# ugovaretto-accel/cuda-mpi-scratch

Hardware: AMD Instinct MI355X
Metric: 2D stencil Gcells/sec (higher is better)
Workload: dtype fp32

## Files before the change

### csrc/include/mxs/kernels/chunk_schedule.hpp

```cpp
#pragma once

#include <algorithm>
#include <cstdint>
#include <stdexcept>
#include <string>
#include <vector>

namespace mxs {
namespace kernels {

struct PassChunk {
  std::int32_t group = 0;
  std::int32_t r0 = 0, r1 = 0;
  std::int32_t pad = 0;
};

struct ChunkSchedule {
  int blocks = 0;
  int entries = 0;
  double bulk_cost = 0;
  std::vector<PassChunk> table;
  const PassChunk& at(int wg, int e) const { return table[size_t(wg) * size_t(entries) + size_t(e)]; }
};

// ... 9 lines not shown
  for (int w = 0; w < blocks && ri < runs.size(); ++w) {
    std::int64_t b = budget(w);
    while (b > fill && ri < runs.size()) {
      const std::int64_t take = std::min(b - fill, runs[ri].r1 - pos);
      emit(w, runs[ri].g, pos, pos + take);
      pos += take;
      b -= take + fill;
      if (pos == runs[ri].r1 && ++ri < runs.size()) pos = runs[ri].r0;
    }
  }
  std::int64_t left = 0;
  for (size_t i = ri; i < runs.size(); ++i) left += runs[i].r1 - (i == ri ? pos : runs[i].r0);
  return left;
}
template <typename BudgetT>
std::int64_t min_budget(const std::vector<Run>& runs, int blocks, std::int64_t fill, BudgetT budget_t) {
  std::int64_t total = 0;
  for (const auto& r : runs) total += r.r1 - r.r0;
  std::int64_t lo = 0, hi = total + 4 * fill + 1;
  auto ok = [&](std::int64_t T) {
    return greedy_walk(runs, blocks, fill, [&](int w) { return budget_t(w, T); },
                       [](int, std::int32_t, std::int64_t, std::int64_t) {}) == 0;
  };
  while (!ok(hi)) hi *= 2;
  while (lo + 1 < hi) {
    const std::int64_t mid = lo + (hi - lo) / 2;
    (ok(mid) ? hi : lo) = mid;
  }
  return hi;
}
}

inline std::vector<std::int64_t> balanced_starts(std::int64_t groups, std::int64_t rows, int blocks,
                                                 std::int64_t fill) {
  std::vector<detail::Run> runs;
  for (std::int64_t g = 0; g < groups; ++g) runs.push_back(detail::Run{std::int32_t(g), 0, rows});
  const std::int64_t T = detail::min_budget(runs, blocks, fill, [](int, std::int64_t t) { return t; });
  std::vector<std::int64_t> start(size_t(blocks) + 1, groups * rows);
  std::vector<std::uint8_t> seen(size_t(blocks), 0);
  detail::greedy_walk(runs, blocks, fill, [&](int) { return T; },
                      [&](int w, std::int32_t g, std::int64_t r0, std::int64_t) {
                        if (!seen[size_t(w)]) {
                          seen[size_t(w)] = 1;
                          start[size_t(w)] = std::int64_t(g) * rows + r0;
                        }
                      });
  for (int w = blocks - 1; w >= 0; --w)
    if (!seen[size_t(w)]) start[size_t(w)] = start[size_t(w) + 1];
  return start;
}

struct HaloLastSchedule {
  ChunkSchedule inner;
  ChunkSchedule outer;
  std::int64_t hf = 0;
  double inner_cost = 0, outer_cost = 0;
  double serial_cost = 0;
  std::int64_t band = 0;
  std::int64_t moved_rows = 0;
};

namespace detail {
inline ChunkSchedule partition_runs(const std::vector<Run>& runs, int blocks, std::int64_t fill, double* cost) {
  ChunkSchedule s;
  s.blocks = blocks;
  std::vector<std::vector<PassChunk>> lists(static_cast<size_t>(blocks));
  std::vector<std::int64_t> load(static_cast<size_t>(blocks), 0);
  if (!runs.empty()) {
    const std::int64_t T = min_budget(runs, blocks, fill, [](int, std::int64_t t) { return t; });
    greedy_walk(runs, blocks, fill, [&](int) { return T; },
                [&](int w, std::int32_t g, std::int64_t r0, std::int64_t r1) {
// ... 151 lines not shown
```

### csrc/include/mxs/kernels/kernels.hpp

```cpp
#pragma once

#include <hip/hip_runtime_api.h>

#include <cmath>
#include <cstdint>
#include <limits>

#include "mxs/grid/layout.hpp"
#include "mxs/kernels/chunk_schedule.hpp"
#include "mxs/kernels/fixed_edge_split.hpp"

namespace mxs {
namespace kernels {

template <typename T>
void fill(T* p, index_t n, T value, hipStream_t s);
template <typename T>
void fill_region(T* base, const Array2D& region, T value, hipStream_t s);
template <typename T>
void fill_random(T* tile, const TileGeom& g, index_t global_x0, index_t global_y0,
                 index_t global_width, std::uint64_t seed, T lo, T hi, hipStream_t s);

struct Stencil5Coeffs {
  double center = 0.2;
// ... 65 lines not shown
  int lag1 = 0;
  int blocks = 0;
  index_t groups = 0;
  index_t owg = 0;
  index_t fill = 0;
  index_t read_lead = 0, read_span = 0;
};
template <typename T>
bool chunk_pass_shape(const TileGeom& g, int steps, const Stencil5Coeffs& c, ChunkPassShape* out);
template <typename T>
void stencil5_chunk_pass(const T* in, T* out, const TileGeom& g, const Stencil5Coeffs& c, const ChunkPassShape& shape,
                         const PassChunk* table, int entries, hipStream_t s);

template <typename T>
void absmax(const T* x, index_t n, T* out, hipStream_t s);
bool streams_concurrent(hipStream_t a, hipStream_t b);
void spin_delay(double us, hipStream_t s);
constexpr int kClockStampWgs = 512;
void clock_stamp(unsigned long long* out, hipStream_t s);
void count_diff(const void* a, const void* b, index_t bytes, unsigned* out, hipStream_t s);

template <typename T>
void stencil5_rect(const T* in, T* out, const TileGeom& g, index_t x0, index_t x1, index_t y0,
                   index_t y1, Stencil5Coeffs c, hipStream_t s);

void set_gpu_share(int processes);
int gpu_share();

void set_pipe_joint(bool on);
bool pipe_joint();
void set_pipe_lag1(bool on);
bool pipe_lag1();
bool last_pipe_lag1();
void set_pipe_balanced(bool on);
bool pipe_balanced_on();

const char* last_stencil_dispatch();

constexpr int kMaxBoxRadius = 2;
struct BoxWeights {
  int radius = 1;
  float w[(2 * kMaxBoxRadius + 1) * (2 * kMaxBoxRadius + 1)] = {};
};
template <typename T>
void stencil_box(const T* in, T* out, const TileGeom& g, index_t x0, index_t x1, index_t y0,
                 index_t y1, const BoxWeights& w, hipStream_t s);

constexpr int kMaxCopies = 24;
struct Copy2D {
  index_t src_off = 0, src_stride = 0;
  index_t dst_off = 0, dst_stride = 0;
  index_t width = 0, height = 0;
  int src_slot = 0, dst_slot = 0;
};
struct Copy2DBatch {
  int n = 0;
  Copy2D op[kMaxCopies];
};
enum class CopyKind : int { Copy = 0, Pack = 1, Unpack = 2 };
template <typename T>
void copy2d_batch(T* slot0, T* slot1, T* slot2, const Copy2DBatch& b, hipStream_t s, int grid_x = 0, int block = 0,
                  CopyKind kind = CopyKind::Copy);

enum class DotReduce : int {
  Atomic = 0,
  TwoPass = 1,
// ... 15 lines not shown
```

### csrc/kernels/stencil.hip

```cpp
#include <hip/hip_runtime.h>

#include <algorithm>
#include <atomic>
#include <cmath>
#include <limits>
#include <cstdlib>
#include <string>
#include <vector>

#include "mxs/core/error.hpp"
#include "mxs/kernels/kernels.hpp"
#include "mxs/runtime/hip_utils.hpp"

#include "stencil_device.hpp"
#include "stencil_pipe.hpp"

namespace mxs {
namespace kernels {
namespace {
using namespace detail;
constexpr int kLdsRows = 16;

std::atomic<const char*> g_last_dispatch{"none"};
std::atomic<bool> g_last_lag1{false};
inline void note(const char* k) {
  g_last_dispatch.store(k, std::memory_order_relaxed);
  g_last_lag1.store(false, std::memory_order_relaxed);
}

template <typename T, int ROWS>
void launch_roll(const T* in, T* out, const TileGeom& g, index_t row_begin, index_t row_end, T c0, T c1,
                 hipStream_t s) {
  constexpr int N = Vec16<T>::N;
  constexpr int WX = 4, NW = 4;
  const index_t rows = row_end - row_begin;
  const index_t gx = (g.width + index_t(kWaveSize) * N * WX - 1) / (index_t(kWaveSize) * N * WX);
  const index_t gy = (rows + ROWS - 1) / ROWS;
  stencil5_roll_kernel<T, ROWS, ROWS, true, WX, false, NW><<<dim3(unsigned(gx), unsigned(gy)), NW * kWaveSize, 0, s>>>(
      in, out, g.pitch, g.core_offset(), g.width, row_begin, row_end, c0, c1);
}

}

template <typename T>
void stencil5_rows(const T* in, T* out, const TileGeom& g, index_t row_begin, index_t row_end,
                   Stencil5Coeffs c, hipStream_t s, StencilVariant v) {
  if (row_end <= row_begin || g.width <= 0) return;
  MXS_CHECK(g.halo_x >= 1 && g.halo_y >= 1, "stencil5 needs a ghost ring of at least 1");
  MXS_CHECK(row_begin >= 0 && row_end <= g.height, "row range out of the core");
  constexpr int N = Vec16<T>::N;
  MXS_CHECK((g.pitch % N) == 0 && ((g.x_origin + g.halo_x) % N) == 0,
            "stencil5_rows needs a TileGeom::aligned layout (16-byte aligned core rows)");
  MXS_CHECK(g.pitch >= g.x_origin + g.halo_x + ((g.width + N - 1) / N) * N + N,
            "pitch too small for vector loads");
  const T c0 = T(c.center), c1 = T(c.neighbor);
  const index_t rows = row_end - row_begin;
  const index_t gx = (g.width + kWaveSize * N - 1) / (kWaveSize * N);
  if (v == StencilVariant::LdsTile) {
    const index_t gy = (rows + kLdsRows - 1) / kLdsRows;
    const size_t lds = size_t(kLdsRows + 2) * (kWaveSize * N + 2 * N) * sizeof(T);
// ... 202 lines not shown
  stencil5_rect_kernel<T><<<unsigned(blocks), kBlock, 0, s>>>(in, out, g.pitch, g.core_offset(), x0, x1 - x0, y0,
                                                              y1 - y0, T(c.center), T(c.neighbor));
  note("rect");
  MXS_HIP_CHECK_LAUNCH();
}

template <typename T>
void stencil_box(const T* in, T* out, const TileGeom& g, index_t x0, index_t x1, index_t y0, index_t y1,
                 const BoxWeights& w, hipStream_t s) {
  if (x1 <= x0 || y1 <= y0) return;
  MXS_CHECK(w.radius == 1 || w.radius == 2, "box radius must be 1 or 2");
  MXS_CHECK(g.halo_x >= w.radius && g.halo_y >= w.radius, "ghost ring narrower than the box radius");
  const dim3 grid(unsigned((x1 - x0 + 63) / 64), unsigned((y1 - y0 + 15) / 16));
  if (w.radius == 1)
    stencil_box_kernel<T, 1><<<grid, kBlock, 0, s>>>(in, out, g.pitch, g.core_offset(), x0, x1 - x0, y0, y1 - y0, w);
  else
    stencil_box_kernel<T, 2><<<grid, kBlock, 0, s>>>(in, out, g.pitch, g.core_offset(), x0, x1 - x0, y0, y1 - y0, w);
  note("box");
  MXS_HIP_CHECK_LAUNCH();
}

const char* last_stencil_dispatch() { return g_last_dispatch.load(std::memory_order_relaxed); }

namespace {
std::atomic<int> g_gpu_share{1};
std::atomic<bool> g_pipe_joint{[] {
  const char* e = experiment_env("MXS_PIPE_JOINT");
  return !(e && std::string(e) == "0");
}()};
std::atomic<bool> g_pipe_lag1{[] {
  const char* e = experiment_env("MXS_PIPE_LAG1");
  return !(e && std::string(e) == "0");
}()};
std::atomic<bool> g_pipe_balanced{[] {
  const char* e = experiment_env("MXS_PIPE_BALANCED");
  return !(e && std::string(e) == "0");
}()};
}
void set_gpu_share(int processes) { g_gpu_share.store(std::max(1, processes), std::memory_order_relaxed); }
int gpu_share() { return g_gpu_share.load(std::memory_order_relaxed); }
void set_pipe_joint(bool on) { g_pipe_joint.store(on, std::memory_order_relaxed); }
bool pipe_joint() { return g_pipe_joint.load(std::memory_order_relaxed); }
void set_pipe_lag1(bool on) { g_pipe_lag1.store(on, std::memory_order_relaxed); }
bool pipe_lag1() { return g_pipe_lag1.load(std::memory_order_relaxed); }
bool last_pipe_lag1() { return g_last_lag1.load(std::memory_order_relaxed); }
void set_pipe_balanced(bool on) { g_pipe_balanced.store(on, std::memory_order_relaxed); }
bool pipe_balanced_on() { return g_pipe_balanced.load(std::memory_order_relaxed); }
namespace detail {
bool pipe_balanced() { return g_pipe_balanced.load(std::memory_order_relaxed); }
void pipe_starts(index_t groups, index_t rows, int blocks, index_t fill, PipeShares* out) {
  struct Entry {
    index_t groups, rows, fill;
    int blocks;
    std::vector<std::int64_t> start;
  };
  thread_local std::vector<Entry> cache;
  const Entry* hit = nullptr;
  for (const auto& e : cache)
    if (e.groups == groups && e.rows == rows && e.fill == fill && e.blocks == blocks) hit = &e;
  if (!hit) {
    if (cache.size() >= 16) cache.erase(cache.begin());
    cache.push_back(Entry{groups, rows, fill, blocks, balanced_starts(groups, rows, blocks, fill)});
    hit = &cache.back();
  }
  out->n = blocks;
  for (int w = 0; w <= blocks; ++w) out->start[w] = int(hit->start[size_t(w)]);
}
void note_dispatch(const char* k) { note(k); }
void note_pipe_lag1(bool lag1) { g_last_lag1.store(lag1, std::memory_order_relaxed); }
}

#define MXS_INST_STENCIL(T)                                                                                    \
  template void stencil5_rows<T>(const T*, T*, const TileGeom&, index_t, index_t, Stencil5Coeffs, hipStream_t, \
                                 StencilVariant);                                                              \
  template void stencil5_rect<T>(const T*, T*, const TileGeom&, index_t, index_t, index_t, index_t,             \
                                 Stencil5Coeffs, hipStream_t);                                                 \
  template void stencil5_periodic<T>(const T*, T*, const TileGeom&, Stencil5Coeffs, hipStream_t);              \
  template void stencil5_tb<T>(const T*, T*, const TileGeom&, int, index_t, index_t, index_t, index_t,          \
                               Stencil5Coeffs, bool, hipStream_t, StencilVariant);                             \
  template bool stencil5_periodic_supported<T>(const TileGeom&);                                               \
  template void stencil_box<T>(const T*, T*, const TileGeom&, index_t, index_t, index_t, index_t,               \
                               const BoxWeights&, hipStream_t);
MXS_INST_STENCIL(float)
MXS_INST_STENCIL(double)

}
}
```

### csrc/kernels/stencil_device.hpp

```cpp
#pragma once

#include <hip/hip_runtime.h>

#include "mxs/kernels/kernels.hpp"

namespace mxs {
namespace kernels {
namespace detail {

template <typename T>
struct Vec16 {
  static constexpr int N = 16 / sizeof(T);
  using type = T __attribute__((ext_vector_type(N)));
};

template <typename T>
__device__ __forceinline__ T fma_t(T a, T b, T c);
template <>
__device__ __forceinline__ float fma_t<float>(float a, float b, float c) { return __builtin_fmaf(a, b, c); }
template <>
__device__ __forceinline__ double fma_t<double>(double a, double b, double c) { return __builtin_fma(a, b, c); }

template <typename T>
__device__ __forceinline__ T jac(T c, T n, T s, T w, T e, T c0, T c1) {
// ... 897 lines not shown
    if (xw < x_end) {
      wp.done = a - a0;
      if constexpr (ROT)
        stream_chunk_fast<typename FastBody<T, SUM, XB>::type, S, PF, WRAP>(in, out, pitch, core_off, W, H, xw, x_end,
                                                                        y_begin + r0, y_begin + r1, c0, c1, &wp);
      else
        stream_chunk<T, S, PF, WRAP, DPP>(in, out, pitch, core_off, W, H, xw, x_end, y_begin + r0, y_begin + r1, c0,
                                          c1);
    }
    a += r1 - r0;
  }
}

template <int S0, int S1, int PF>
struct PipeShape {
  static constexpr int S = S0 + S1;
  static constexpr int RING = 3 * PF;
  static constexpr int T1 = (3 * S0 + PF - 1 + PF - 1) / PF;
};

template <int S0, int S1, int G>
struct JointShape {
  static constexpr int A0 = (S0 + 3) / 4 * 4, A1 = (S1 + 3) / 4 * 4;
  static constexpr int OW0 = 256 - 2 * A0;
  static constexpr int OW1 = 256 - 2 * A1;
  static constexpr int SPAN = G * OW0;
  static constexpr int OWG = SPAN - 2 * A1 < G * OW1 ? SPAN - 2 * A1 : G * OW1;
  static constexpr int ROW = G * kWaveSize;
  static constexpr int LEAD = A0 + A1;
  static_assert((G - 1) * OW1 + 256 <= 4 * ROW, "stage-1 windows must stay inside the joint row");
  static_assert(OWG > 0, "time block too deep for a joint group");
};

template <typename B, int S0, int S1, int PF, bool WRAP, bool JOINT = false, int G = kWavesPerBlock, int LAG1 = 0>
__device__ __forceinline__ void pipe_chunk(const typename B::T* __restrict__ in, typename B::T* __restrict__ out,
                                           index_t pitch, index_t core_off, index_t W, index_t H, index_t xw,
                                           index_t x_end, index_t ys, index_t ye, typename B::T c0, typename B::T c1,
                                           typename B::V* __restrict__ ring, int stage, int strip = 0) {
  static_assert(PF % 3 == 0, "the window rotates through 3 slots: PF must be a multiple of 3");
  using P = PipeShape<S0, S1, PF>;
  constexpr int S = P::S, RING = P::RING;
  using T = typename B::T;
  using V = typename B::V;
  using Sh = StripShape<T, S, true>;
  using J = JointShape<S0, S1, G>;
  constexpr bool ASC0 = (LAG1 & 1) != 0, ASC1 = (LAG1 & 2) != 0;
  constexpr int E0 = ASC0 ? 2 * S0 : 3 * S0 - 1, E1 = ASC1 ? 2 * S1 : 3 * S1 - 1;
  constexpr int N = Sh::N, SA = Sh::SA, AL = SA / N;
  static_assert(!JOINT || N == 4, "joint windows assume 4-cell lanes");
  const int lane = threadIdx.x & (kWaveSize - 1);
  const index_t gx = JOINT ? (stage == 0 ? xw - J::LEAD + index_t(strip) * J::OW0 : xw - J::A1 + index_t(strip) * J::OW1) +
                                 index_t(lane) * N
                           : xw - SA + index_t(lane) * N;
  const index_t rows = ye - ys;
  constexpr int D = (PF - E0 % PF) % PF;
  constexpr int T1 = (E0 + D) / PF + 1;
  static_assert(ASC0 || T1 == P::T1, "stage-1 start block");
  const index_t n_it0 = rows + 2 * S1 + E0 + D;
  const index_t n_it1 = rows + E1;
  const index_t blocks0 = (n_it0 + PF - 1) / PF, blocks1 = T1 + (n_it1 + PF - 1) / PF;
  const index_t blocks = blocks0 > blocks1 ? blocks0 : blocks1;
  constexpr int RSTRIDE = JOINT ? J::ROW : kWaveSize;
  int slot = lane;
  if constexpr (JOINT) {
    constexpr int AL0 = J::A0 / 4;
    if (stage == 0) {
      const bool valid = lane >= AL0 && lane < kWaveSize - AL0;
      const int tail = J::SPAN / 4 + strip * 2 * AL0 + (lane < AL0 ? lane : lane - (kWaveSize - 2 * AL0));
      slot = valid ? strip * (J::OW0 / 4) + lane - AL0 : tail;
    } else {
      slot = strip * (J::OW1 / 4) + lane;
    }
  }
  V* __restrict__ my = ring + slot;

  if (stage == 0) {
    index_t lx;
    if (!JOINT && xw >= x_end) {
      lx = 0;
    } else if constexpr (WRAP) {
      if (W >= (JOINT ? G : 1) * kWaveSize * N) lx = gx < 0 ? gx + W : (gx >= W ? gx - W : gx);
      else lx = ((gx % W) + W) % W;
    } else {
      const index_t last_col = (W + N - 1) / N * N + SA - N;
      lx = gx < last_col ? gx : last_col;
    }
    const T* __restrict__ pin = in + core_off + lx;
    const index_t last_row = ye + S - 1;
    V pf[PF];
#pragma unroll
    for (int k = 0; k < PF; ++k) {
      index_t r = ys - S - D + k;
      if constexpr (WRAP) r = r < 0 ? r + H : r;
      else r = r < ys - S ? ys - S : r;
      pf[k] = B::load(pin + r * pitch);
    }
    index_t next = ys - S - D + PF;
    if constexpr (WRAP) next = next < 0 ? next + H : next;
    index_t roff = next * pitch;
    auto fetch = [&]() -> V {
      const V v = B::load(pin + roff);
// ... 55 lines not shown
            if (l == S0 - 1) top = v;
            else win[n][l + 1] = v;
          }
        } else {
          const int p0 = k % 3, p1 = (k + 1) % 3, p2 = (k + 2) % 3;
          win[p2][0] = B::enter(pf[k]);
          pf[k] = fetch();
#pragma unroll
          for (int l = S0 - 1; l >= 0; --l) {
            const V o = B::jac(win[p0][l], win[p1][l], win[p2][l], c0, c1);
            if (l == S0 - 1) top = o;
            else win[p0][l + 1] = o;
          }
        }
        my[(base + k) * RSTRIDE] = top;
        if constexpr (B::kStage0Fence) __builtin_amdgcn_sched_barrier(0);
      }
      base = base + PF < RING ? base + PF : 0;
      __syncthreads();
    }
  } else {
    const index_t x0w = gx - index_t(lane) * N;
    const T* obase = out + core_off + x0w + ys * pitch;
    const unsigned long long ob = reinterpret_cast<unsigned long long>(obase);
    const unsigned ob_lo = __builtin_amdgcn_readfirstlane(unsigned(ob)),
                   ob_hi = __builtin_amdgcn_readfirstlane(unsigned(ob >> 32));
    T* obase_u = reinterpret_cast<T*>((static_cast<unsigned long long>(ob_hi) << 32) | ob_lo);
    const int nbytes = __builtin_amdgcn_readfirstlane(int(rows * pitch * index_t(sizeof(T))));
    const __amdgpu_buffer_rsrc_t orsrc = __builtin_amdgcn_make_buffer_rsrc(obase_u, 0, nbytes, 0x00020000);
    bool store_lane;
    if constexpr (JOINT) {
      constexpr int AL1 = J::A1 / 4;
      const int q = strip * J::OW1 + lane * N;
      store_lane = lane >= AL1 && lane < kWaveSize - AL1 && q + N <= J::A1 + J::OWG && gx < x_end;
    } else {
      store_lane = lane >= AL && lane < kWaveSize - AL && gx < x_end && xw < x_end;
    }
    const unsigned lane_term = store_lane ? unsigned(lane) * unsigned(N * sizeof(T)) : 0x80000000u;
    const unsigned row_bytes = unsigned(pitch) * unsigned(sizeof(T));
    const int rows_i = int(rows);
    V win[3][S1];
#pragma unroll
    for (int q = 0; q < 3; ++q)
#pragma unroll
      for (int l = 0; l < S1; ++l) win[q][l] = B::zero();
#pragma unroll 1
    for (int t = 0; t < T1; ++t) __syncthreads();
    constexpr int kWarm = ASC1 ? (2 * S1) / PF * PF : (3 * (S1 - 1)) / PF * PF;
#pragma unroll 1
    for (int ib = 0; ib < kWarm; ib += PF) {
      V inrow[PF];
      const int base = (ib / PF) % 3 * PF;
#pragma unroll
      for (int k = 0; k < PF; ++k) inrow[k] = my[(base + k) * RSTRIDE];
#pragma unroll
      for (int k = 0; k < PF; ++k) {
        if constexpr (ASC1) {
          const int n = k % 3, o = (k + 1) % 3, m = (k + 2) % 3;
          const int b = (ib + k) / 2;
          win[n][0] = inrow[k];
#pragma unroll
          for (int l = 0; l < S1 - 1; ++l)
            if (l < b) win[n][l + 1] = B::jac(win[o][l], win[m][l], win[n][l], c0, c1);
        } else {
          const int p0 = k % 3, p1 = (k + 1) % 3, p2 = (k + 2) % 3;
          const int b = (ib + k) / 3;
          win[p2][0] = inrow[k];
// ... 13 lines not shown
      base = base + PF < RING ? base + PF : 0;
#pragma unroll
      for (int k = 0; k < PF; ++k) {
        const index_t j = i + k;
        V top;
        if constexpr (ASC1) {
          const int n = k % 3, o = (k + 1) % 3, m = (k + 2) % 3;
          win[n][0] = inrow[k];
#pragma unroll
          for (int l = 0; l < S1; ++l) {
            const V v = B::jac(win[o][l], win[m][l], win[n][l], c0, c1);
            if (l == S1 - 1) top = v;
            else win[n][l + 1] = v;
          }
        } else {
          const int p0 = k % 3, p1 = (k + 1) % 3, p2 = (k + 2) % 3;
          win[p2][0] = inrow[k];
#pragma unroll
          for (int l = S1 - 1; l >= 0; --l) {
            const V o = B::jac(win[p0][l], win[p1][l], win[p2][l], c0, c1);
            if (l == S1 - 1) top = o;
            else win[p0][l + 1] = o;
          }
        }
        const int r = int(j - E1);
        const unsigned row_term = r >= 0 && r < rows_i ? unsigned(r) * row_bytes : unsigned(kMaxChunkBytes);
        B::store(top, orsrc, lane_term + row_term, c0);
      }
      __syncthreads();
    }
  }
}

constexpr int kMaxShareBlocks = 512;
struct PipeShares {
  index_t share = 0;
  int n = 0;
  int start[kMaxShareBlocks + 1];
  static PipeShares equal(index_t share) {
    PipeShares p;
    p.share = share;
    return p;
  }
};

template <int S0, int S1, int PF, bool WRAP, int PRIO = 0, typename T = float, bool SUM = false,
          int G = kWavesPerBlock, bool XM = false, bool JOINT = false, int LAG1 = 0, int XB = 0>
__global__ __launch_bounds__(2 * G * kWaveSize) void stencil5_stream_pipe_kernel(
    const T* __restrict__ in, T* __restrict__ out, index_t pitch, index_t core_off, index_t W, index_t H,
    index_t x_begin, index_t x_end, index_t y_begin, index_t y_end, const PipeShares shares, T c0, T c1) {
  using P = PipeShape<S0, S1, PF>;
  using B = typename FastBody<T, SUM, XB>::type;
  constexpr int OW = StripShape<T, P::S, true>::OW;
  constexpr int OWG = JointShape<S0, S1, G>::OWG;
  __shared__ typename B::V ring[G * P::RING * kWaveSize];
  const index_t rows = y_end - y_begin;
  const index_t strips = (x_end - x_begin + OW - 1) / OW;
  const index_t groups = JOINT ? (x_end - x_begin + OWG - 1) / OWG : (strips + G - 1) / G;
  const index_t total = groups * rows;
  const int wave = threadIdx.x / kWaveSize;
  const int strip = wave % G, stage = wave / G;
  if constexpr (PRIO == 1) {
    if (stage == 0) __builtin_amdgcn_s_setprio(1);
  } else if constexpr (PRIO == 2) {
    if (stage == 1) __builtin_amdgcn_s_setprio(1);
  }
  index_t slot = blockIdx.x;
  if constexpr (XM) {
    if (gridDim.x % kNumXcds == 0) slot = (blockIdx.x % kNumXcds) * (gridDim.x / kNumXcds) + blockIdx.x / kNumXcds;
  }
  index_t a, b;
  if (shares.n > 0) {
    a = shares.start[slot];
    b = shares.start[slot + 1];
  } else {
    a = slot * shares.share;
    b = a + shares.share < total ? a + shares.share : total;
  }
  const index_t max_rows = kMaxChunkBytes / (pitch * index_t(sizeof(T)));
  if (max_rows < 1) return;
#pragma unroll 1
  while (a < b) {
    const index_t grp = a / rows, r0 = a - grp * rows;
    index_t r1 = rows < r0 + (b - a) ? rows : r0 + (b - a);
    r1 = r1 - r0 > max_rows ? r0 + max_rows : r1;
    if constexpr (JOINT) {
      pipe_chunk<B, S0, S1, PF, WRAP, true, G, LAG1>(in, out, pitch, core_off, W, H, x_begin + grp * OWG, x_end,
                                               y_begin + r0, y_begin + r1, c0, c1, ring, stage, strip);
    } else {
      const index_t xw = x_begin + (grp * G + strip) * OW;
      pipe_chunk<B, S0, S1, PF, WRAP, false, G, LAG1>(in, out, pitch, core_off, W, H, xw, x_end, y_begin + r0, y_begin + r1, c0, c1,
                                      ring + strip * P::RING * kWaveSize, stage);
    }
    a += r1 - r0;
  }
}

template <int S0, int S1, int PF, typename T, bool SUM, int LAG1, int XB = 0>
__global__ __launch_bounds__(2 * kWavesPerBlock * kWaveSize) void stencil5_pipe_chunks_kernel(
    const T* __restrict__ in, T* __restrict__ out, index_t pitch, index_t core_off, index_t W, index_t H,
    index_t x_begin, index_t x_end, index_t y_begin, const PassChunk* __restrict__ table, int entries, T c0, T c1) {
  constexpr int G = kWavesPerBlock;
  using P = PipeShape<S0, S1, PF>;
  using B = typename FastBody<T, SUM, XB>::type;
  constexpr int OWG = JointShape<S0, S1, G>::OWG;
  __shared__ typename B::V ring[G * P::RING * kWaveSize];
  const int wave = threadIdx.x / kWaveSize;
  const int strip = wave % G, stage = wave / G;
  const PassChunk* __restrict__ mine = table + index_t(blockIdx.x) * entries;
  const index_t max_rows = kMaxChunkBytes / (pitch * index_t(sizeof(T)));
  if (max_rows < 1) return;
#pragma unroll 1
  for (int e = 0; e < entries; ++e) {
    const PassChunk c = mine[e];
    if (c.r1 <= c.r0) break;
#pragma unroll 1
    for (index_t r0 = c.r0; r0 < c.r1; r0 += max_rows) {
      const index_t r1 = c.r1 - r0 > max_rows ? r0 + max_rows : c.r1;
      pipe_chunk<B, S0, S1, PF, false, true, G, LAG1>(in, out, pitch, core_off, W, H, x_begin + index_t(c.group) * OWG,
                                                     x_end, y_begin + r0, y_begin + r1, c0, c1, ring, stage, strip);
    }
  }
}

}
// ... 3 lines not shown
```

### csrc/kernels/stencil_pipe.hpp

```cpp
#pragma once

#include <algorithm>

#include "mxs/core/error.hpp"
#include "mxs/kernels/kernels.hpp"
#include "mxs/runtime/hip_utils.hpp"
#include "stencil_device.hpp"

namespace mxs {
namespace kernels {
namespace detail {

void note_dispatch(const char* kernel);
void note_pipe_lag1(bool lag1);

constexpr int kPipeMinF64 = 9;

template <typename T, int S, bool SUM>
constexpr int pipe_s0() {
  if constexpr (sizeof(T) == 8 || SUM) return S / 2;
  return S / 2 + 1 < 16 ? S / 2 + 1 : 16;
}
template <typename T, int S>
constexpr int pipe_pf() {
  return (sizeof(T) == 4 && S <= 28) ? 6 : 3;
}
template <typename T, int S>
constexpr bool pipe_joint_ok() {
  return sizeof(T) == 4 ? (S % 4 == 0 && S >= 20) : S == 16;
}
template <typename T, int S>
constexpr int joint_s0() {
  return sizeof(T) == 8 ? S / 2 : (S >= 32 ? 16 : 12);
}
constexpr index_t kLag1MaxChunk = index_t(1) << 62;
constexpr int kLagBoth = 3;
constexpr index_t kLag1MaxChunkF64 = index_t(1) << 62;
constexpr index_t kJointWide = 12288;

template <typename T, int S, bool WRAP, bool SUM, int JS0 = 0, int LAG1 = 0, int XB = 0>
constexpr auto pipe_kernel() {
  if constexpr (JS0 > 0)
    return stencil5_stream_pipe_kernel<JS0, S - JS0, pipe_pf<T, S>(), WRAP, 0, T, SUM, kWavesPerBlock, false, true,
                                       LAG1, XB>;
  else
    return stencil5_stream_pipe_kernel<pipe_s0<T, S, SUM>(), S - pipe_s0<T, S, SUM>(), pipe_pf<T, S>(), WRAP, 0, T,
                                       SUM>;
}

template <typename T, int S, bool WRAP, bool SUM, int JS0 = 0>
int pipe_blocks() {
  static int blocks = 0;
  if (blocks == 0) {
    int occ = 0;
    MXS_HIP_CHECK(hipOccupancyMaxActiveBlocksPerMultiprocessor(
        &occ, reinterpret_cast<const void*>(pipe_kernel<T, S, WRAP, SUM, JS0>()), 2 * kBlock, 0));
    blocks = std::max(occ, 1) * device_cu_count();
  }
  return std::max(1, blocks / gpu_share());
}

template <typename T, int S, bool WRAP, bool SUM, int JS0 = 0>
index_t pipe_share(index_t x0, index_t x1, index_t y0, index_t y1) {
  constexpr int OW = StripShape<T, S, true>::OW;
  constexpr int OWG = JointShape<(JS0 > 0 ? JS0 : S / 2), S - (JS0 > 0 ? JS0 : S / 2), kWavesPerBlock>::OWG;
  const index_t groups =
      JS0 > 0 ? (x1 - x0 + OWG - 1) / OWG : ((x1 - x0 + OW - 1) / OW + kWavesPerBlock - 1) / kWavesPerBlock;
  const int blocks = pipe_blocks<T, S, WRAP, SUM, JS0>();
  return (groups * (y1 - y0) + blocks - 1) / blocks;
}

template <int S0, int S1, int PF, int LAG1>
constexpr index_t pipe_fill_rows() {
  constexpr bool A0 = (LAG1 & 1) != 0, A1 = (LAG1 & 2) != 0;
  constexpr int E0 = A0 ? 2 * S0 : 3 * S0 - 1, E1 = A1 ? 2 * S1 : 3 * S1 - 1;
  constexpr int D = (PF - E0 % PF) % PF;
  constexpr int T1 = (E0 + D) / PF + 1;
  constexpr int a = 2 * S1 + E0 + D, b = T1 * PF + E1;
  return (a > b ? a : b) + PF - 1;
}

void pipe_starts(index_t groups, index_t rows, int blocks, index_t fill, PipeShares* out);

bool pipe_balanced();

template <typename T, int S, bool WRAP, bool SUM, int JS0, int LAG1 = 0, int XB = 0>
void launch_pipe_form(const T* in, T* out, const TileGeom& g, index_t x0, index_t x1, index_t y0, index_t y1, T c0,
                      T c1, T sc, hipStream_t s) {
  static_assert(XB == 0 || (SUM && XB == kScaledBody && JS0 > 0), "the scaled form runs the joint pipeline");
  const index_t share = pipe_share<T, S, WRAP, SUM, JS0>(x0, x1, y0, y1);
  const int blocks = pipe_blocks<T, S, WRAP, SUM, JS0>();
  PipeShares shares = PipeShares::equal(share);
  if (pipe_balanced() && blocks <= kMaxShareBlocks) {
    constexpr int S0 = JS0 > 0 ? JS0 : pipe_s0<T, S, SUM>();
    constexpr int OW = StripShape<T, S, true>::OW;
    constexpr int OWG = JointShape<(JS0 > 0 ? JS0 : S / 2), S - (JS0 > 0 ? JS0 : S / 2), kWavesPerBlock>::OWG;
    const index_t groups =
        JS0 > 0 ? (x1 - x0 + OWG - 1) / OWG : ((x1 - x0 + OW - 1) / OW + kWavesPerBlock - 1) / kWavesPerBlock;
    pipe_starts(groups, y1 - y0, blocks, pipe_fill_rows<S0, S - S0, pipe_pf<T, S>(), LAG1>(), &shares);
  }
  MXS_CHECK(g.pitch * index_t(sizeof(T)) * kMinChunkRows <= kMaxChunkBytes,
            "stencil5_tb: rows of " << g.pitch * index_t(sizeof(T)) << " bytes leave fewer than " << kMinChunkRows
                                    << " rows per pipeline chunk (buffer-descriptor stores)");
  const T kc = XB == kScaledBody ? T(double(c0) / double(c1)) : c1;
  pipe_kernel<T, S, WRAP, SUM, JS0, LAG1, XB>()<<<blocks, 2 * kBlock, 0, s>>>(
      in, out, g.pitch, g.core_offset(), g.width, g.height, x0, x1, y0, y1, shares, SUM ? sc : c0, kc);
  note_dispatch(XB == kScaledBody ? "stream_pipe_scaled" : SUM ? "stream_pipe_sum" : "stream_pipe");
  note_pipe_lag1(LAG1 != 0);
}

template <typename T, int S, bool WRAP, bool SUM, int XB = 0>
void launch_pipe_impl(const T* in, T* out, const TileGeom& g, index_t x0, index_t x1, index_t y0, index_t y1, T c0, T c1,
                 T sc, hipStream_t s) {
  if constexpr (pipe_joint_ok<T, S>()) {
    if (pipe_joint()) {
      if constexpr (sizeof(T) == 4 && S == 20) {
        if (pipe_lag1() && pipe_share<T, S, WRAP, SUM, 12>(x0, x1, y0, y1) <= kLag1MaxChunk) {
          if (x1 - x0 < kJointWide)
            return launch_pipe_form<T, S, WRAP, SUM, 8, kLagBoth, XB>(in, out, g, x0, x1, y0, y1, c0, c1, sc, s);
          return launch_pipe_form<T, S, WRAP, SUM, 12, kLagBoth, XB>(in, out, g, x0, x1, y0, y1, c0, c1, sc, s);
        }
      } else if constexpr (sizeof(T) == 4 && S == 24) {
        if (pipe_lag1())
          return launch_pipe_form<T, S, WRAP, SUM, 12, kLagBoth, XB>(in, out, g, x0, x1, y0, y1, c0, c1, sc, s);
      } else if constexpr (sizeof(T) == 8 && S == 16) {
        if (pipe_lag1() && pipe_share<T, S, WRAP, SUM, 8>(x0, x1, y0, y1) <= kLag1MaxChunkF64)
          return launch_pipe_form<T, S, WRAP, SUM, 8, kLagBoth, XB>(in, out, g, x0, x1, y0, y1, c0, c1, sc, s);
      }
      return launch_pipe_form<T, S, WRAP, SUM, joint_s0<T, S>(), 0, XB>(in, out, g, x0, x1, y0, y1, c0, c1, sc, s);
    }
  }
  if constexpr (XB == 0) {
    launch_pipe_form<T, S, WRAP, SUM, 0>(in, out, g, x0, x1, y0, y1, c0, c1, sc, s);
  } else {
    launch_pipe_form<T, S, WRAP, false, 0>(in, out, g, x0, x1, y0, y1, c0, c1, sc, s);
  }
}

template <typename T, int S, bool WRAP>
bool wide_pipe_ok_impl(const TileGeom& g, index_t x0, index_t x1, index_t y0, index_t y1) {
  constexpr int SA = StripShape<T, S, true>::SA;
// ... 20 lines not shown
```

### csrc/python/bind_core.cpp

```cpp
#include <pybind11/pybind11.h>
#include <pybind11/stl.h>

#include <sstream>

#include "mxs/core/error.hpp"
#include "mxs/grid/layout.hpp"
#include "mxs/grid/regions.hpp"
#include "mxs/halo/plan.hpp"
#include "mxs/kernels/chunk_schedule.hpp"
#include "mxs/kernels/fixed_edge_split.hpp"
#include "mxs/runtime/decision.hpp"
#include "mxs/topo/cart.hpp"

namespace py = pybind11;
using namespace mxs;

PYBIND11_MODULE(_mxs_core, m) {
  m.doc() = "mxs host-side core: layouts, regions, Cartesian topology, halo plans";

  py::class_<Array2D>(m, "Array2D")
      .def(py::init<index_t, index_t, index_t, index_t, index_t>(), py::arg("width"), py::arg("height"),
           py::arg("row_stride"), py::arg("x_offset") = 0, py::arg("y_offset") = 0)
      .def_readwrite("width", &Array2D::width)
      .def_readwrite("height", &Array2D::height)
// ... 177 lines not shown
        out["notch"] = d.notch;
        out["serial_ms"] = d.baseline_ms;
        out["candidate_ms"] = d.candidate_ms;
        out["ratios"] = d.ratios;
        return out;
      },
      py::arg("serial"), py::arg("candidates"), py::arg("min_gain") = 0.0, py::arg("rule") = "median",
      "StencilSolver::choose_opening's collective rule: per-round maxima over ranks, paired ratios of the maxima, "
      "the lowest notch among candidates, which wins when its median ratio is <= 1 - min_gain (rule 'median', the "
      "opening) or its notch is below it (rule 'notch', the steady and direct-halo decisions) "
      "(runtime/decision.hpp); missing slots: kMissingSample");
  m.attr("MISSING_SAMPLE") = kMissingSample;
  m.attr("HOLD_TOP") = unsigned(kernels::kHoldTop);
  m.attr("HOLD_BOTTOM") = unsigned(kernels::kHoldBottom);
  m.attr("HOLD_LEFT") = unsigned(kernels::kHoldLeft);
  m.attr("HOLD_RIGHT") = unsigned(kernels::kHoldRight);
  m.def(
      "fixed_edge_split",
      [](index_t w, index_t h, int S, int vec, unsigned hold) {
        const kernels::FixedEdgeSplit sp = kernels::fixed_edge_split(w, h, S, vec, hold);
        auto rect = [](const kernels::Rect& r) { return py::make_tuple(r.x0, r.x1, r.y0, r.y1); };
        py::list frame;
        for (int i = 0; i < sp.n_frame; ++i) frame.append(rect(sp.frame[i]));
        py::dict d;
        d["interior"] = rect(sp.interior);
        d["frame"] = frame;
        return d;
      },
      py::arg("width"), py::arg("height"), py::arg("steps"), py::arg("vec"), py::arg("hold"),
      "time blocking beside fixed edges: the core's interior (x0, x1, y0, y1), shrunk by `steps` on the held sides "
      "(HOLD_* bits; left / right to whole `vec`-cell vectors), and the frame rectangles that cover the rest "
      "(kernels/fixed_edge_split.hpp); an empty interior is (0, 0, 0, 0)");
  m.def("balanced_starts", &kernels::balanced_starts, py::arg("groups"), py::arg("rows"), py::arg("blocks"),
        py::arg("fill"), "fill-aware linear starts of the pipeline workgroups' shares (blocks + 1 entries)");
  m.def(
      "halo_last_schedule",
      [](std::int64_t groups, std::int64_t rows, int blocks, std::int64_t fill, std::int64_t depth,
         std::vector<std::uint8_t> ghost, int outer_wgs, double lead_frac, std::int64_t band_rows, int granule, int min_outer) {
        const auto h = kernels::make_halo_last_schedule(groups, rows, blocks, fill, depth, ghost, outer_wgs, lead_frac,
                                                        band_rows, granule, min_outer);
        auto lists = [](const kernels::ChunkSchedule& s) {
          py::list table;
          for (int w = 0; w < s.blocks; ++w) {
            py::list l;
            for (int e = 0; e < s.entries; ++e) {
              const auto& c = s.at(w, e);
              if (c.r1 > c.r0) l.append(py::make_tuple(c.group, c.r0, c.r1));
            }
            table.append(l);
          }
          return table;
        };
        py::dict d;
        d["inner"] = lists(h.inner);
        d["outer"] = lists(h.outer);
        d["hf"] = h.hf;
        d["inner_cost"] = h.inner_cost;
        d["outer_cost"] = h.outer_cost;
        d["serial_cost"] = h.serial_cost;
        d["moved_rows"] = h.moved_rows;
        d["band"] = h.band;
        d["check"] = kernels::check_halo_last_schedule(h, groups, rows, depth, ghost);
        return d;
      },
      py::arg("groups"), py::arg("rows"), py::arg("blocks"), py::arg("fill"), py::arg("depth"), py::arg("ghost"),
      py::arg("outer_wgs") = 0, py::arg("lead_frac") = 0.12, py::arg("band_rows") = 0, py::arg("granule") = 1,
      py::arg("min_outer") = 1,
// ... 3 lines not shown
```

### csrc/python/bind_hip.cpp

```cpp
#include <pybind11/pybind11.h>
#include <pybind11/stl.h>

#include <memory>
#include <stdexcept>
#include <string>

#include "mxs/comm/rccl_comm.hpp"
#include "mxs/core/fault.hpp"
#include "mxs/halo/exchange.hpp"
#include "mxs/kernels/kernels.hpp"
#include "mxs/runtime/ipc.hpp"
#include "mxs/runtime/pingpong.hpp"
#include "mxs/runtime/stencil_solver.hpp"

namespace py = pybind11;
using namespace mxs;

namespace {

template <typename T>
T* ptr(std::uintptr_t p) {
  return reinterpret_cast<T*>(p);
}
hipStream_t strm(std::uintptr_t s) { return reinterpret_cast<hipStream_t>(s); }
// ... 111 lines not shown
         const std::string& dt, std::uintptr_t s, const std::string& variant) {
        kernels::Stencil5Coeffs c{c0, c1};
        const auto v = parse_variant(variant);
        if (parse_dtype(dt) == DType::F32)
          kernels::stencil5_rows<float>(ptr<float>(in), ptr<float>(out), g, r0, r1, c, strm(s), v);
        else
          kernels::stencil5_rows<double>(ptr<double>(in), ptr<double>(out), g, r0, r1, c, strm(s), v);
      },
      py::arg("src"), py::arg("dst"), py::arg("geom"), py::arg("row_begin"), py::arg("row_end"),
      py::arg("c_center") = 0.2, py::arg("c_neighbor") = 0.2, py::arg("dtype") = "f32", py::arg("stream") = 0,
      py::arg("variant") = "auto");
  m.def(
      "auto_time_block",
      [](index_t w, index_t h, const std::string& dt, bool sum_form) {
        return kernels::auto_time_block(w, h, parse_dtype(dt) == DType::F32 ? 4 : 8, sum_form);
      },
      py::arg("width"), py::arg("height"), py::arg("dtype") = "f32", py::arg("sum_form") = true,
      "measured default Jacobi steps per pass / halo exchange for a tile");
  m.attr("MAX_TIME_BLOCK") = kernels::kMaxTimeBlock;
  m.attr("MAX_TIME_BLOCK_DEEP") = kernels::kMaxTimeBlockDeep;
  m.def(
      "last_stencil_dispatch", [] { return std::string(kernels::last_stencil_dispatch()); },
      "kernel form chosen by the most recent stencil launcher (e.g. 'stream_balanced_rot')");
  m.def("device_cu_count", &device_cu_count, "compute units of the current HIP device");
  m.def("set_gpu_share", &kernels::set_gpu_share, py::arg("processes"),
        "processes sharing this GPU: persistent stencil kernels take 1/processes of the chip");
  m.def("gpu_share", &kernels::gpu_share);
  m.def("set_pipe_joint", &kernels::set_pipe_joint, py::arg("on"),
        "joint stage-1 windows in the fp32 two-stage pipeline (default on; bitwise equal output)");
  m.def("pipe_joint", &kernels::pipe_joint);
  m.def("set_pipe_lag1", &kernels::set_pipe_lag1, py::arg("on"),
        "ascending level order in the joint fp32 pipeline where it pays (default on; bitwise equal output)");
  m.def("pipe_lag1", &kernels::pipe_lag1);
  m.def("set_pipe_balanced", &kernels::set_pipe_balanced, py::arg("on"),
        "fill-aware workgroup shares in the pipeline passes (default on; bitwise equal output)");
  m.def("pipe_balanced", &kernels::pipe_balanced_on);
  m.def(
      "absmax",
      [](std::uintptr_t x, index_t n, const std::string& dt) {
        double r = 0;
        if (parse_dtype(dt) == DType::F32) {
          DeviceBuffer<float> o(1);
          kernels::absmax<float>(ptr<float>(x), n, o.get(), nullptr);
          float h = 0;
          MXS_HIP_CHECK(hipMemcpy(&h, o.get(), sizeof(float), hipMemcpyDeviceToHost));
          r = h;
        } else {
          DeviceBuffer<double> o(1);
          kernels::absmax<double>(ptr<double>(x), n, o.get(), nullptr);
          MXS_HIP_CHECK(hipMemcpy(&r, o.get(), sizeof(double), hipMemcpyDeviceToHost));
        }
        return r;
      },
      py::arg("x"), py::arg("n"), py::arg("dtype") = "f32", "max |x[i]| (device reduction; NaN if any is NaN)");
  m.def(
      "stencil5_chunk_pass",
      [](std::uintptr_t in, std::uintptr_t out, const TileGeom& g, int steps, double c0, double c1,
         const std::string& dt, int outer_wgs, std::uintptr_t s, bool sum_form, double range, double lead_frac,
         const std::string& part) -> py::object {
        MXS_CHECK(part == "both" || part == "inner" || part == "outer", "stencil5_chunk_pass: part both|inner|outer");
        kernels::Stencil5Coeffs c{c0, c1, sum_form, range};
        auto run = [&](auto tag) -> py::object {
          using T = decltype(tag);
          kernels::ChunkPassShape sh;
          if (!kernels::chunk_pass_shape<T>(g, steps, c, &sh) || sh.blocks < 2) return py::none();
          std::vector<std::uint8_t> ghost(size_t(sh.groups), 0);
// ... 573 lines not shown
```

Before: 11530.

## Split narrow last column group into two half-height sub-groups in joint pipeline

When the last column group of the fp32 S=24 joint pipeline is narrow enough to fit in half a workgroup's width, the pass now cuts it into two sub-groups of two waves each. Each sub-group processes half of the rows, so that group's row count, and the share scheduling built on it, is roughly halved. The goal is to remove the load imbalance and wasted lanes caused by a mostly empty final group. In exchange it adds a new special-case code path with wave-uniform row offsets, split ring usage, and a balanced-start computation that has to account for the shorter last run.

```diff
diff --git a/csrc/include/mxs/kernels/chunk_schedule.hpp b/csrc/include/mxs/kernels/chunk_schedule.hpp
--- a/csrc/include/mxs/kernels/chunk_schedule.hpp
+++ b/csrc/include/mxs/kernels/chunk_schedule.hpp
@@ -65,11 +65,13 @@
 }
 
 inline std::vector<std::int64_t> balanced_starts(std::int64_t groups, std::int64_t rows, int blocks,
-                                                 std::int64_t fill) {
+                                                 std::int64_t fill, std::int64_t last_rows = 0) {
+  if (last_rows <= 0 || last_rows > rows) last_rows = rows;
   std::vector<detail::Run> runs;
-  for (std::int64_t g = 0; g < groups; ++g) runs.push_back(detail::Run{std::int32_t(g), 0, rows});
+  for (std::int64_t g = 0; g < groups; ++g)
+    runs.push_back(detail::Run{std::int32_t(g), 0, g + 1 == groups ? last_rows : rows});
   const std::int64_t T = detail::min_budget(runs, blocks, fill, [](int, std::int64_t t) { return t; });
-  std::vector<std::int64_t> start(size_t(blocks) + 1, groups * rows);
+  std::vector<std::int64_t> start(size_t(blocks) + 1, (groups - 1) * rows + last_rows);
   std::vector<std::uint8_t> seen(size_t(blocks), 0);
   detail::greedy_walk(runs, blocks, fill, [&](int) { return T; },
                       [&](int w, std::int32_t g, std::int64_t r0, std::int64_t) {
diff --git a/csrc/include/mxs/kernels/kernels.hpp b/csrc/include/mxs/kernels/kernels.hpp
--- a/csrc/include/mxs/kernels/kernels.hpp
+++ b/csrc/include/mxs/kernels/kernels.hpp
@@ -121,6 +121,9 @@
 void set_pipe_lag1(bool on);
 bool pipe_lag1();
 bool last_pipe_lag1();
+void set_pipe_split(bool on);
+bool pipe_split();
+bool last_pipe_split();
 void set_pipe_balanced(bool on);
 bool pipe_balanced_on();
 
diff --git a/csrc/kernels/stencil.hip b/csrc/kernels/stencil.hip
--- a/csrc/kernels/stencil.hip
+++ b/csrc/kernels/stencil.hip
@@ -23,9 +23,11 @@
 
 std::atomic<const char*> g_last_dispatch{"none"};
 std::atomic<bool> g_last_lag1{false};
+std::atomic<bool> g_last_split{false};
 inline void note(const char* k) {
   g_last_dispatch.store(k, std::memory_order_relaxed);
   g_last_lag1.store(false, std::memory_order_relaxed);
+  g_last_split.store(false, std::memory_order_relaxed);
 }
 
 template <typename T, int ROWS>
@@ -294,6 +296,10 @@
   const char* e = experiment_env("MXS_PIPE_LAG1");
   return !(e && std::string(e) == "0");
 }()};
+std::atomic<bool> g_pipe_split{[] {
+  const char* e = experiment_env("MXS_PIPE_SPLIT");
+  return !(e && std::string(e) == "0");
+}()};
 std::atomic<bool> g_pipe_balanced{[] {
   const char* e = experiment_env("MXS_PIPE_BALANCED");
   return !(e && std::string(e) == "0");
@@ -306,23 +312,27 @@
 void set_pipe_lag1(bool on) { g_pipe_lag1.store(on, std::memory_order_relaxed); }
 bool pipe_lag1() { return g_pipe_lag1.load(std::memory_order_relaxed); }
 bool last_pipe_lag1() { return g_last_lag1.load(std::memory_order_relaxed); }
+void set_pipe_split(bool on) { g_pipe_split.store(on, std::memory_order_relaxed); }
+bool pipe_split() { return g_pipe_split.load(std::memory_order_relaxed); }
+bool last_pipe_split() { return g_last_split.load(std::memory_order_relaxed); }
 void set_pipe_balanced(bool on) { g_pipe_balanced.store(on, std::memory_order_relaxed); }
 bool pipe_balanced_on() { return g_pipe_balanced.load(std::memory_order_relaxed); }
 namespace detail {
 bool pipe_balanced() { return g_pipe_balanced.load(std::memory_order_relaxed); }
-void pipe_starts(index_t groups, index_t rows, int blocks, index_t fill, PipeShares* out) {
+void pipe_starts(index_t groups, index_t rows, int blocks, index_t fill, PipeShares* out, index_t last_rows) {
   struct Entry {
-    index_t groups, rows, fill;
+    index_t groups, rows, fill, last_rows;
     int blocks;
     std::vector<std::int64_t> start;
   };
   thread_local std::vector<Entry> cache;
   const Entry* hit = nullptr;
   for (const auto& e : cache)
-    if (e.groups == groups && e.rows == rows && e.fill == fill && e.blocks == blocks) hit = &e;
+    if (e.groups == groups && e.rows == rows && e.fill == fill && e.last_rows == last_rows && e.blocks == blocks)
+      hit = &e;
   if (!hit) {
     if (cache.size() >= 16) cache.erase(cache.begin());
-    cache.push_back(Entry{groups, rows, fill, blocks, balanced_starts(groups, rows, blocks, fill)});
+    cache.push_back(Entry{groups, rows, fill, last_rows, blocks, balanced_starts(groups, rows, blocks, fill, last_rows)});
     hit = &cache.back();
   }
   out->n = blocks;
@@ -330,6 +340,7 @@
 }
 void note_dispatch(const char* k) { note(k); }
 void note_pipe_lag1(bool lag1) { g_last_lag1.store(lag1, std::memory_order_relaxed); }
+void note_pipe_split(bool split) { g_last_split.store(split, std::memory_order_relaxed); }
 }
 
 #define MXS_INST_STENCIL(T)                                                                                    \
diff --git a/csrc/kernels/stencil_device.hpp b/csrc/kernels/stencil_device.hpp
--- a/csrc/kernels/stencil_device.hpp
+++ b/csrc/kernels/stencil_device.hpp
@@ -953,11 +953,14 @@
   static_assert(OWG > 0, "time block too deep for a joint group");
 };
 
-template <typename B, int S0, int S1, int PF, bool WRAP, bool JOINT = false, int G = kWavesPerBlock, int LAG1 = 0>
+template <typename B, int S0, int S1, int PF, bool WRAP, bool JOINT = false, int G = kWavesPerBlock, int LAG1 = 0,
+          bool SUB = false>
 __device__ __forceinline__ void pipe_chunk(const typename B::T* __restrict__ in, typename B::T* __restrict__ out,
                                            index_t pitch, index_t core_off, index_t W, index_t H, index_t xw,
                                            index_t x_end, index_t ys, index_t ye, typename B::T c0, typename B::T c1,
-                                           typename B::V* __restrict__ ring, int stage, int strip = 0) {
+                                           typename B::V* __restrict__ ring, int stage, int strip = 0,
+                                           index_t sync_rows = 0, int gs = G) {
+  static_assert(!SUB || JOINT, "sub-groups are cut from joint windows");
   static_assert(PF % 3 == 0, "the window rotates through 3 slots: PF must be a multiple of 3");
   using P = PipeShape<S0, S1, PF>;
   constexpr int S = P::S, RING = P::RING;
@@ -977,8 +980,11 @@
   constexpr int D = (PF - E0 % PF) % PF;
   constexpr int T1 = (E0 + D) / PF + 1;
   static_assert(ASC0 || T1 == P::T1, "stage-1 start block");
-  const index_t n_it0 = rows + 2 * S1 + E0 + D;
-  const index_t n_it1 = rows + E1;
+  const index_t brows = SUB ? sync_rows : rows;
+  const int span = SUB ? gs * J::OW0 : J::SPAN;
+  const int owg = SUB ? (span - 2 * J::A1 < gs * J::OW1 ? span - 2 * J::A1 : gs * J::OW1) : J::OWG;
+  const index_t n_it0 = brows + 2 * S1 + E0 + D;
+  const index_t n_it1 = brows + E1;
   const index_t blocks0 = (n_it0 + PF - 1) / PF, blocks1 = T1 + (n_it1 + PF - 1) / PF;
   const index_t blocks = blocks0 > blocks1 ? blocks0 : blocks1;
   constexpr int RSTRIDE = JOINT ? J::ROW : kWaveSize;
@@ -987,7 +993,7 @@
     constexpr int AL0 = J::A0 / 4;
     if (stage == 0) {
       const bool valid = lane >= AL0 && lane < kWaveSize - AL0;
-      const int tail = J::SPAN / 4 + strip * 2 * AL0 + (lane < AL0 ? lane : lane - (kWaveSize - 2 * AL0));
+      const int tail = span / 4 + strip * 2 * AL0 + (lane < AL0 ? lane : lane - (kWaveSize - 2 * AL0));
       slot = valid ? strip * (J::OW0 / 4) + lane - AL0 : tail;
     } else {
       slot = strip * (J::OW1 / 4) + lane;
@@ -1109,7 +1115,7 @@
     if constexpr (JOINT) {
       constexpr int AL1 = J::A1 / 4;
       const int q = strip * J::OW1 + lane * N;
-      store_lane = lane >= AL1 && lane < kWaveSize - AL1 && q + N <= J::A1 + J::OWG && gx < x_end;
+      store_lane = lane >= AL1 && lane < kWaveSize - AL1 && q + N <= J::A1 + owg && gx < x_end;
     } else {
       store_lane = lane >= AL && lane < kWaveSize - AL && gx < x_end && xw < x_end;
     }
@@ -1189,9 +1195,20 @@
   }
 }
 
+__device__ __forceinline__ int wave_uniform(int v) { return __builtin_amdgcn_readfirstlane(v); }
+__device__ __forceinline__ index_t wave_uniform(index_t v) {
+  const unsigned long long u = static_cast<unsigned long long>(v);
+  const unsigned lo = __builtin_amdgcn_readfirstlane(unsigned(u)), hi = __builtin_amdgcn_readfirstlane(unsigned(u >> 32));
+  return index_t((static_cast<unsigned long long>(hi) << 32) | lo);
+}
+template <typename T, int S0, int S1, int G, bool JOINT, int LAG1>
+constexpr bool pipe_split_form() {
+  return JOINT && sizeof(T) == 4 && G == 4 && S0 == 12 && S1 == 12 && LAG1 == 3;
+}
 constexpr int kMaxShareBlocks = 512;
 struct PipeShares {
   index_t share = 0;
+  index_t split_half = 0;
   int n = 0;
   int start[kMaxShareBlocks + 1];
   static PipeShares equal(index_t share) {
@@ -1214,7 +1231,9 @@
   const index_t rows = y_end - y_begin;
   const index_t strips = (x_end - x_begin + OW - 1) / OW;
   const index_t groups = JOINT ? (x_end - x_begin + OWG - 1) / OWG : (strips + G - 1) / G;
-  const index_t total = groups * rows;
+  constexpr bool SPLIT = pipe_split_form<T, S0, S1, G, JOINT, LAG1>();
+  const index_t half = SPLIT ? shares.split_half : 0;
+  const index_t total = half > 0 ? (groups - 1) * rows + half : groups * rows;
   const int wave = threadIdx.x / kWaveSize;
   const int strip = wave % G, stage = wave / G;
   if constexpr (PRIO == 1) {
@@ -1239,15 +1258,31 @@
 #pragma unroll 1
   while (a < b) {
     const index_t grp = a / rows, r0 = a - grp * rows;
+    if constexpr (SPLIT) {
+      if (half > 0 && grp == groups - 1) {
+        index_t r1 = half < r0 + (b - a) ? half : r0 + (b - a);
+        r1 = r1 - r0 > max_rows ? r0 + max_rows : r1;
+        const int sub = wave_uniform(strip / 2), sstrip = wave_uniform(strip % 2);
+        const index_t q0 = wave_uniform(!sub ? r0 : r0 + half < rows ? r0 + half : rows);
+        const index_t q1 = wave_uniform(!sub ? r1 : r1 + half < rows ? r1 + half : rows);
+        using J = JointShape<S0, S1, G>;
+        static_assert(JointShape<S0, S1, G / 2>::ROW * 2 == J::ROW, "a sub-group's joint row is half the ring row");
+        pipe_chunk<B, S0, S1, PF, WRAP, true, G, LAG1, true>(in, out, pitch, core_off, W, H, x_begin + grp * OWG, x_end,
+                                                             y_begin + q0, y_begin + q1, c0, c1,
+                                                             ring + sub * (J::ROW / 2), stage, sstrip, r1 - r0, G / 2);
+        a += r1 - r0;
+        continue;
+      }
+    }
     index_t r1 = rows < r0 + (b - a) ? rows : r0 + (b - a);
     r1 = r1 - r0 > max_rows ? r0 + max_rows : r1;
     if constexpr (JOINT) {
       pipe_chunk<B, S0, S1, PF, WRAP, true, G, LAG1>(in, out, pitch, core_off, W, H, x_begin + grp * OWG, x_end,
-                                               y_begin + r0, y_begin + r1, c0, c1, ring, stage, strip);
+                                                     y_begin + r0, y_begin + r1, c0, c1, ring, stage, strip);
     } else {
       const index_t xw = x_begin + (grp * G + strip) * OW;
-      pipe_chunk<B, S0, S1, PF, WRAP, false, G, LAG1>(in, out, pitch, core_off, W, H, xw, x_end, y_begin + r0, y_begin + r1, c0, c1,
-                                      ring + strip * P::RING * kWaveSize, stage);
+      pipe_chunk<B, S0, S1, PF, WRAP, false, G, LAG1>(in, out, pitch, core_off, W, H, xw, x_end, y_begin + r0,
+                                                      y_begin + r1, c0, c1, ring + strip * P::RING * kWaveSize, stage);
     }
     a += r1 - r0;
   }
diff --git a/csrc/kernels/stencil_pipe.hpp b/csrc/kernels/stencil_pipe.hpp
--- a/csrc/kernels/stencil_pipe.hpp
+++ b/csrc/kernels/stencil_pipe.hpp
@@ -13,6 +13,7 @@
 
 void note_dispatch(const char* kernel);
 void note_pipe_lag1(bool lag1);
+void note_pipe_split(bool split);
 
 constexpr int kPipeMinF64 = 9;
 
@@ -60,14 +61,32 @@
   return std::max(1, blocks / gpu_share());
 }
 
-template <typename T, int S, bool WRAP, bool SUM, int JS0 = 0>
-index_t pipe_share(index_t x0, index_t x1, index_t y0, index_t y1) {
+template <typename T, int S, int JS0 = 0>
+index_t pipe_groups(index_t x0, index_t x1) {
   constexpr int OW = StripShape<T, S, true>::OW;
   constexpr int OWG = JointShape<(JS0 > 0 ? JS0 : S / 2), S - (JS0 > 0 ? JS0 : S / 2), kWavesPerBlock>::OWG;
-  const index_t groups =
-      JS0 > 0 ? (x1 - x0 + OWG - 1) / OWG : ((x1 - x0 + OW - 1) / OW + kWavesPerBlock - 1) / kWavesPerBlock;
+  return JS0 > 0 ? (x1 - x0 + OWG - 1) / OWG : ((x1 - x0 + OW - 1) / OW + kWavesPerBlock - 1) / kWavesPerBlock;
+}
+
+template <typename T, int S, int JS0, int LAG1>
+index_t pipe_split_half(index_t x0, index_t x1, index_t y0, index_t y1) {
+  if constexpr (JS0 > 0) {
+    if constexpr (pipe_split_form<T, JS0, S - JS0, kWavesPerBlock, true, LAG1>()) {
+      constexpr int OWG = JointShape<JS0, S - JS0, kWavesPerBlock>::OWG;
+      constexpr int OWG2 = JointShape<JS0, S - JS0, 2>::OWG;
+      const index_t rem = (x1 - x0) - (pipe_groups<T, S, JS0>(x0, x1) - 1) * OWG;
+      if (pipe_split() && rem <= OWG2) return (y1 - y0 + 1) / 2;
+    }
+  }
+  return 0;
+}
+
+template <typename T, int S, bool WRAP, bool SUM, int JS0 = 0>
+index_t pipe_share(index_t x0, index_t x1, index_t y0, index_t y1, index_t split_half = 0) {
+  const index_t groups = pipe_groups<T, S, JS0>(x0, x1);
   const int blocks = pipe_blocks<T, S, WRAP, SUM, JS0>();
-  return (groups * (y1 - y0) + blocks - 1) / blocks;
+  const index_t total = split_half > 0 ? (groups - 1) * (y1 - y0) + split_half : groups * (y1 - y0);
+  return (total + blocks - 1) / blocks;
 }
 
 template <int S0, int S1, int PF, int LAG1>
@@ -80,7 +99,7 @@
   return (a > b ? a : b) + PF - 1;
 }
 
-void pipe_starts(index_t groups, index_t rows, int blocks, index_t fill, PipeShares* out);
+void pipe_starts(index_t groups, index_t rows, int blocks, index_t fill, PipeShares* out, index_t last_rows = 0);
 
 bool pipe_balanced();
 
@@ -88,16 +107,15 @@
 void launch_pipe_form(const T* in, T* out, const TileGeom& g, index_t x0, index_t x1, index_t y0, index_t y1, T c0,
                       T c1, T sc, hipStream_t s) {
   static_assert(XB == 0 || (SUM && XB == kScaledBody && JS0 > 0), "the scaled form runs the joint pipeline");
-  const index_t share = pipe_share<T, S, WRAP, SUM, JS0>(x0, x1, y0, y1);
+  const index_t split_half = pipe_split_half<T, S, JS0, LAG1>(x0, x1, y0, y1);
+  const index_t share = pipe_share<T, S, WRAP, SUM, JS0>(x0, x1, y0, y1, split_half);
   const int blocks = pipe_blocks<T, S, WRAP, SUM, JS0>();
   PipeShares shares = PipeShares::equal(share);
+  shares.split_half = split_half;
   if (pipe_balanced() && blocks <= kMaxShareBlocks) {
     constexpr int S0 = JS0 > 0 ? JS0 : pipe_s0<T, S, SUM>();
-    constexpr int OW = StripShape<T, S, true>::OW;
-    constexpr int OWG = JointShape<(JS0 > 0 ? JS0 : S / 2), S - (JS0 > 0 ? JS0 : S / 2), kWavesPerBlock>::OWG;
-    const index_t groups =
-        JS0 > 0 ? (x1 - x0 + OWG - 1) / OWG : ((x1 - x0 + OW - 1) / OW + kWavesPerBlock - 1) / kWavesPerBlock;
-    pipe_starts(groups, y1 - y0, blocks, pipe_fill_rows<S0, S - S0, pipe_pf<T, S>(), LAG1>(), &shares);
+    pipe_starts(pipe_groups<T, S, JS0>(x0, x1), y1 - y0, blocks, pipe_fill_rows<S0, S - S0, pipe_pf<T, S>(), LAG1>(),
+                &shares, split_half);
   }
   MXS_CHECK(g.pitch * index_t(sizeof(T)) * kMinChunkRows <= kMaxChunkBytes,
             "stencil5_tb: rows of " << g.pitch * index_t(sizeof(T)) << " bytes leave fewer than " << kMinChunkRows
@@ -107,6 +125,7 @@
       in, out, g.pitch, g.core_offset(), g.width, g.height, x0, x1, y0, y1, shares, SUM ? sc : c0, kc);
   note_dispatch(XB == kScaledBody ? "stream_pipe_scaled" : SUM ? "stream_pipe_sum" : "stream_pipe");
   note_pipe_lag1(LAG1 != 0);
+  note_pipe_split(split_half > 0);
 }
 
 template <typename T, int S, bool WRAP, bool SUM, int XB = 0>
diff --git a/csrc/python/bind_core.cpp b/csrc/python/bind_core.cpp
--- a/csrc/python/bind_core.cpp
+++ b/csrc/python/bind_core.cpp
@@ -233,7 +233,9 @@
       "(HOLD_* bits; left / right to whole `vec`-cell vectors), and the frame rectangles that cover the rest "
       "(kernels/fixed_edge_split.hpp); an empty interior is (0, 0, 0, 0)");
   m.def("balanced_starts", &kernels::balanced_starts, py::arg("groups"), py::arg("rows"), py::arg("blocks"),
-        py::arg("fill"), "fill-aware linear starts of the pipeline workgroups' shares (blocks + 1 entries)");
+        py::arg("fill"), py::arg("last_rows") = 0,
+        "fill-aware linear starts of the pipeline workgroups' shares (blocks + 1 entries); last_rows > 0: the last "
+        "group's run is that long (the split narrow group), 0 = rows");
   m.def(
       "halo_last_schedule",
       [](std::int64_t groups, std::int64_t rows, int blocks, std::int64_t fill, std::int64_t depth,
diff --git a/csrc/python/bind_hip.cpp b/csrc/python/bind_hip.cpp
--- a/csrc/python/bind_hip.cpp
+++ b/csrc/python/bind_hip.cpp
@@ -167,6 +167,12 @@
   m.def("set_pipe_lag1", &kernels::set_pipe_lag1, py::arg("on"),
         "ascending level order in the joint fp32 pipeline where it pays (default on; bitwise equal output)");
   m.def("pipe_lag1", &kernels::pipe_lag1);
+  m.def("set_pipe_split", &kernels::set_pipe_split, py::arg("on"),
+        "split a narrow last column group of the fp32 S = 24 pass into two half-height sub-groups (default on; "
+        "bitwise equal output)");
+  m.def("pipe_split", &kernels::pipe_split);
+  m.def("last_pipe_split", &kernels::last_pipe_split,
+        "whether the most recent stencil launch was a pipeline pass that split its last group");
   m.def("set_pipe_balanced", &kernels::set_pipe_balanced, py::arg("on"),
         "fill-aware workgroup shares in the pipeline passes (default on; bitwise equal output)");
   m.def("pipe_balanced", &kernels::pipe_balanced_on);
```

Measured after the change: 11710 (median of 6 runs). 1.02x the previous value.
